# mbjd/binaural-audio-synthesis

Measured on AMD Instinct MI355X. Metric: stereo samples/sec, 256 concurrent moving sources @44.1kHz mixed to one stereo pair (x real-time in x_realtime), higher is better.
Workload: dtype f32

## Files before the change

binaural-audio-synthesis_amd/csrc/bas_fused.h:

```cpp
#pragma once
#include "bas_internal.h"
#include "bas_plan.h"
#include "bas_window.h"
#include "bas_tail.h"

#ifndef FZ_ASM
#define FZ_ASM 1
#endif
#if FZ_ASM
#ifndef BAS_FIR_ASM_INC
#define BAS_FIR_ASM_INC "bas_fir_asm.inc"
#endif
#include BAS_FIR_ASM_INC
#ifndef BAS_FIR_ONCE_ASM_INC
#define BAS_FIR_ONCE_ASM_INC "bas_fir_once_asm.inc"
#endif
#include BAS_FIR_ONCE_ASM_INC
#else
template <int XR>
__device__ __forceinline__ void ffa_row_step_asm(f32x32 &, f32x32 &, f32x2 &, f32x32 &, unsigned, unsigned, float, unsigned) {}
#endif

struct FzArgs {
    long x_stride;
    int n_src;
    long T_in;
    int K, S, L, Lp;
    int n_chunks;
    int s_pow2;
    float invK, invS;
    long units_total;
    int units_per_wg, parts_per_wg;
    int nslots;
    int spw;
    unsigned packed_bytes;
    int direct;
    int accumulate;
    long T_out;
    unsigned *ctl;
    int tail_mode;
#ifdef BAS_DIAG
    int inject;
#endif
};

__device__ __forceinline__ bool fz_wait_handover(volatile unsigned *flag, unsigned pass_id, const FzArgs &A) {
    int limit = 1 << 22;
#ifdef BAS_DIAG
    if (A.inject) limit = 1 << 8;
#endif
    int spins = 0;
    while ((unsigned)__builtin_amdgcn_readfirstlane(*flag) != pass_id) {
        if (++spins >= limit) {
            if ((threadIdx.x & 63) == 0 && A.ctl) bas_report_status(A.ctl, BAS_STATUS_HANDOVER_TIMEOUT, blockIdx.x);
            return false;
        }
        __builtin_amdgcn_s_sleep(1);
    }
    return true;
}

__device__ __forceinline__ bool fz_inject(const FzArgs &A) {
#ifdef BAS_DIAG
    return A.inject != 0;
#else
    return false;
#endif
}

__device__ __forceinline__ BasTail fz_tail(const FzArgs &A, float *y, unsigned int *peak_bits) {
    BasTail T;
    T.ctl = A.ctl;
    T.wgpeak = reinterpret_cast<float *>(A.ctl + BAS_CTL_WORDS);
    T.y = y;
    T.n = 2 * A.T_out;
    T.peak = reinterpret_cast<float *>(peak_bits);
    T.n_wg = gridDim.x;
    T.normalize = 0;
    return T;
}

__device__ __forceinline__ void fz_pair_ears(const f32x4 &h, f32x2 &ta, f32x2 &tb) {
    const auto s0 = __builtin_amdgcn_permlane32_swap(__float_as_uint(h.z), __float_as_uint(h.x), false, false);
    const auto s1 = __builtin_amdgcn_permlane32_swap(__float_as_uint(h.w), __float_as_uint(h.y), false, false);
    ta = f32x2{__uint_as_float(s0[0]), __uint_as_float(s0[1])};
    tb = f32x2{__uint_as_float(s1[0]), __uint_as_float(s1[1])};
}


#ifndef FS_UNIT_BLOCK
#define FS_UNIT_BLOCK 1
#endif
#define BAS_FS_MAXEV 6
size_t bas_fs_lds_bytes(int nslots);
int bas_fs_unit_len(int Lp);
hipError_t bas_fs_launch(const FzArgs &A, const float *x, float *slab, const float *packed, const unsigned *plans, float *y,
                         unsigned int *peak_bits, int n_wg, size_t lds_bytes, hipStream_t st, hipEvent_t eb, hipEvent_t ee);

#define BAS_FQ_MAXEV 3
size_t bas_fq_lds_bytes(int nslots);
hipError_t bas_fq_launch(const FzArgs &A, const float *x, float *slab, const float *packed, const unsigned *plans, float *y,
                         unsigned int *peak_bits, int n_wg, size_t lds_bytes, hipStream_t st, hipEvent_t eb, hipEvent_t ee);
```

binaural-audio-synthesis_amd/csrc/bas_fused_split.hip:

```cpp
#include "bas_fused.h"
#include <stdlib.h>

#ifndef FS_PSPLIT
#define FS_PSPLIT 1
#endif
#ifndef FS_TAPS_ONCE
#define FS_TAPS_ONCE 1
#endif
#ifndef FS_STAGER_PRIO
#define FS_STAGER_PRIO 3
#endif
#ifndef FS_FILTER_PRIO
#define FS_FILTER_PRIO 0
#endif

#ifdef BAS_STAMPS
__device__ unsigned long long bas_fs_stamps[1024 * 8 * 8];
#define FS_NOW() __builtin_amdgcn_s_memrealtime()
#else
#define FS_NOW() 0ull
#endif

#if FZ_ASM
template <int UNITLEN, int NSUB = 1, int PSPLIT = 0>
__global__ __launch_bounds__(512, 1) void bas_render_fs_kernel(
    FzArgs A, const float *__restrict__ x,
    float *__restrict__ slab,
    const float *__restrict__ packed,
    const unsigned *__restrict__ plans,
    float *__restrict__ y, unsigned int *__restrict__ peak_bits) {
    constexpr int NW = 4;
    constexpr int THREADS = 64 * NW;
    constexpr int TILE = 2048 * NW;
    constexpr int ROWS = TILE / 32 + HD_HALO;
    constexpr int XR = ROWS + 1;
    constexpr int NX = (ROWS * 8 + THREADS - 1) / THREADS;
    constexpr int XFLOATS = 8 * XR * 4;
    constexpr int MAXEV = BAS_FS_MAXEV;
    constexpr int PL4 = WIN_PL4;
    constexpr int NPV = (MAXEV * PL4 + 63) / 64;
    static_assert(XR == 261, "bas_fir_asm.inc holds the row step for this x-image stride");
    extern __shared__ f32x4 lds4[];
    const int buf4 = (XFLOATS + ((A.nslots * HD_SLOT + 3) & ~3)) / 4;
    f32x4 *pl_base = lds4 + 2 * buf4;
    f32x4 *bnd = pl_base + NW * (MAXEV * PL4);
    volatile unsigned *flags = reinterpret_cast<volatile unsigned *>(bnd + NW * 64);

    const int tid0 = threadIdx.x;
    const int lane0 = tid0 & 63;
    const int wv8 = __builtin_amdgcn_readfirstlane(tid0 >> 6);
    const bool stager = wv8 >= NW;
    const int wv = wv8 & (NW - 1);

    const WinWalk W = win_walk(A.units_total, A.units_per_wg, A.Lp);
    const long n_pass = W.n_pass;
    if (!A.direct && peak_bits && blockIdx.x == 0 && tid0 == 0) *peak_bits = 0u;
    if (n_pass <= 0) {
        if (A.direct && A.tail_mode) bas_tail<2 * THREADS>(fz_tail(A, y, peak_bits), 0.f);
        return;
    }
    unsigned wmax_bits = 0u;
    if (tid0 < NW) flags[tid0] = 0u;
    __syncthreads();

    const long first_tile = W.unit0 / A.n_src;
    long tile = first_tile;
    int s = (int)(W.unit0 - first_tile * A.n_src);
    int sg = 0;
    WinGeo G = win_geo<TILE>(tile, sg, A.K, A.Lp);
    auto advance = [&]() {
        const WinPos N = win_next(tile, s, sg, W.nseg, A.n_src);
        if (N.tile != tile || N.sg != sg) G = win_geo<TILE>(N.tile, N.sg, A.K, A.Lp);
        tile = N.tile, s = N.s, sg = N.sg;
    };
#ifdef BAS_STAMPS
    unsigned long long st_work = 0, st_wait = 0, st_clk = 0;
    const unsigned long long st_begin = FS_NOW(), st_begin_clk = __builtin_amdgcn_s_memtime();
#endif

    if (!stager) {
        if (FS_FILTER_PRIO) __builtin_amdgcn_s_setprio(FS_FILTER_PRIO);
        static_assert(!PSPLIT || (NSUB == 1 && UNITLEN != 0), "the P split exists for the unit blocks of subchunks >= 32");
        f32x32 accA, accB, accP;
        f32x2 accB16 = f32x2{0.f, 0.f};
        f32x16 accPA, accPB, accPP;
        f32x2 accPB8 = f32x2{0.f, 0.f};
#pragma unroll
        for (int i = 0; i < 32; ++i) accA[i] = accB[i] = accP[i] = 0.f;
#pragma unroll
        for (int i = 0; i < 16; ++i) accPA[i] = accPB[i] = accPP[i] = 0.f;
        float *slab_wg = slab + (long)blockIdx.x * A.parts_per_wg * 2 * TILE;
        auto flush = [&](long t) {
            f32x2 acc[32];
            if constexpr (PSPLIT) {
#pragma unroll
                for (int r = 0; r < 8; ++r) {
                    const f32x2 a = f32x2{accPA[2 * r], accPA[2 * r + 1]}, b0 = f32x2{accPB[2 * r], accPB[2 * r + 1]};
                    const f32x2 b1 = r < 7 ? f32x2{accPB[2 * r + 2], accPB[2 * r + 3]} : accPB8;
                    const f32x2 pp = f32x2{accPP[2 * r], accPP[2 * r + 1]};
                    const f32x2 pe = a + b0, po = (pp - a) - b1;
                    accP[4 * r] = pe.x; accP[4 * r + 1] = pe.y;
                    accP[4 * r + 2] = po.x; accP[4 * r + 3] = po.y;
                }
            }
            win_combine_pinned(acc, accA, accB, accB16, accP);
            win_zero_pinned(accA, accB, accB16, accP);
            if constexpr (PSPLIT) {
#pragma unroll
                for (int i = 0; i < 16; ++i) accPA[i] = accPB[i] = accPP[i] = 0.f;
                accPB8 = f32x2{0.f, 0.f};
            }
            if (A.direct) {
                const long n0 = t * TILE + 2048 * wv + 32 * lane0;
                const float lmax = win_store_row_direct(acc, y, A.T_out, n0, A.accumulate);
                if (A.tail_mode) {
                    const unsigned b = win_wave_max_bits(lmax);
                    wmax_bits = b > wmax_bits ? b : wmax_bits;
                } else if (peak_bits) {
                    bas_wave_peak_max(lmax, peak_bits);
                }
                return;
            }
            win_store_row_slab(acc, slab_wg + (t - first_tile) * 2 * TILE + 2048 * wv + 32 * lane0, TILE);
        };
        long open_tile = -1;
        long addr_tile = -1;
        int addr_buf = 0;
        unsigned tapv[5] = {0u, 0u, 0u, 0u, 0u}, xrow4 = 0u;
        float alv[5] = {0.f, 0.f, 0.f, 0.f, 0.f}, blv[5] = {0.f, 0.f, 0.f, 0.f, 0.f};
        float wnv[4] = {0.f, 0.f, 0.f, 0.f};
        const unsigned buf_bytes = 16u * (unsigned)buf4;
        for (long pid = 0; pid < n_pass; ++pid) {
            int tid = tid0;
            asm volatile("" : "+v"(tid));
            const int lane = tid & 63;
#ifdef BAS_STAMPS
            const unsigned long long t0 = FS_NOW();
#endif
            if (tile != open_tile) {
                if (open_tile >= 0) flush(open_tile);
                open_tile = tile;
            }
            if constexpr (UNITLEN != 0) {
                const int cur_buf = (int)(pid & 1);
                const long akey = tile * W.nseg + sg;
                if (akey == addr_tile && cur_buf != addr_buf) {
                    const unsigned delta = cur_buf ? buf_bytes : 0u - buf_bytes;
#pragma unroll
                    for (int r = 0; r < 5; ++r) tapv[r] += delta;
                    xrow4 += delta;
                    addr_buf = cur_buf;
                }
                if (akey != addr_tile) {
                    addr_tile = akey;
                    addr_buf = cur_buf;
                    const unsigned bufb = (unsigned)reinterpret_cast<uintptr_t>(lds4 + cur_buf * buf4);
                    const int row_out = 64 * wv + lane + G.halo;
                    int sl, m_in;
                    win_row_slot(G.mo0 + 32 * row_out, A.K, A.invK, sl, m_in);
                    xrow4 = bufb + 16u * (unsigned)(row_out - 4);
                    unsigned tap = bufb + 4u * (unsigned)(XFLOATS + sl * HD_SLOT - 32 * 4);
#pragma unroll
                    for (int r = 0; r < 5; ++r) {
                        alv[r] = win_weight(m_in, A.S, A.s_pow2, A.invK, A.invS);
                        if constexpr (NSUB == 2) blv[r] = win_weight(m_in + 16, A.S, A.s_pow2, A.invK, A.invS);
                        tapv[r] = tap;
                        m_in -= 32;
                        const bool wrap = m_in < 0;
                        if constexpr (PSPLIT == 2) { if (r < 4) wnv[r] = wrap ? 1.f : alv[r]; }
                        m_in += wrap ? A.K : 0;
                        tap += 32u * 16u - (wrap ? 4u * (unsigned)HD_SLOT : 0u);
                    }
                }
            }
#ifdef BAS_STAMPS
            const unsigned long long t1 = FS_NOW();
#endif
            __syncthreads();
#ifdef BAS_STAMPS
            const unsigned long long t2 = FS_NOW();
#endif
            const f32x4 *xs4 = lds4 + (pid & 1) * buf4;
            const float *hd = reinterpret_cast<const float *>(xs4) + XFLOATS;
            const int Lseg = G.Lseg, halo = G.halo;
#ifdef BAS_STAMPS
            const unsigned long long c0 = __builtin_amdgcn_s_memtime();
#endif
            if constexpr (UNITLEN != 0) {
                if constexpr (PSPLIT == 2) {
                    const unsigned tapo[4] = {tapv[1], tapv[2], tapv[3], tapv[4]};
                    const float wov[4] = {alv[1], alv[2], alv[3], alv[4]};
                    ffa_unitp1_asm<XR, UNITLEN>(accA, accB, accPA, accPB, accPB8, accPP, accB16, xrow4, tapo, wnv, wov);
                } else if constexpr (PSPLIT)
                    ffa_unitp_asm<XR, UNITLEN>(accA, accB, accPA, accPB, accPB8, accPP, accB16, xrow4, tapv, alv);
                else if constexpr (NSUB == 4)
                    ffa_unit4_asm<XR, UNITLEN>(accA, accB, accB16, accP, xrow4, tapv, alv, (float)A.S * A.invK);
                else if constexpr (NSUB == 2)
                    ffa_unit2_asm<XR, UNITLEN>(accA, accB, accB16, accP, xrow4, tapv, alv, blv);
                else
                    ffa_unit_asm<XR, UNITLEN>(accA, accB, accB16, accP, xrow4, tapv, alv);
                (void)hd; (void)Lseg; (void)halo;
            } else {
                const int row_out = 64 * wv + lane + halo;
                int sl, m_in;
                win_row_slot(G.mo0 + 32 * row_out, A.K, A.invK, sl, m_in);
                const f32x4 *xrow = xs4 + row_out;
#pragma unroll 1
                for (int rp = 0; rp <= halo; ++rp) {
                    const float al = win_weight(m_in, A.S, A.s_pow2, A.invK, A.invS);
                    const unsigned mk = win_octet_mask(rp, Lseg);
                    ffa_row_step_asm<XR>(accA, accB, accB16, accP, (unsigned)reinterpret_cast<uintptr_t>(xrow),
                                         (unsigned)reinterpret_cast<uintptr_t>(hd + sl * HD_SLOT + (32 * rp - 32) * 4), al, mk);
                    xrow -= 1;
                    win_row_up(A.K, sl, m_in);
                }
            }
#ifdef BAS_STAMPS
            st_clk += __builtin_amdgcn_s_memtime() - c0;
            st_work += (t1 - t0) + (FS_NOW() - t2);
            st_wait += t2 - t1;
#endif
            advance();
        }
        flush(open_tile);
    } else {
        __builtin_amdgcn_s_setprio(FS_STAGER_PRIO);
        const __amdgpu_buffer_rsrc_t tab =
            __builtin_amdgcn_make_buffer_rsrc(const_cast<float *>(packed), 0, (int)A.packed_bytes, 0x00020000);
        const unsigned L4 = 4u * (unsigned)A.L;
        const int n_ir = A.nslots + 1, base = n_ir / NW, rem = n_ir - base * NW;
        const int slot_a = rfl(wv * base + (wv < rem ? wv : rem));
        const int slot_b = rfl(slot_a + base + (wv < rem ? 1 : 0));
        const int n_ev = slot_a < slot_b ? slot_b - slot_a : 0;
        const bool need_next = n_ev > 0 && slot_b <= A.nslots;
        f32x4 *plw = pl_base + wv * (MAXEV * PL4);
        const int tid = tid0 - THREADS;
        const int lane = tid & 63;
        const int half = lane >> 5;
        const int tq = 4 * (lane & 31) + (lane < 32 ? 2 : 0);
        const unsigned v16 = 16u * (unsigned)tid, l16 = 16u * (unsigned)lane;
        const bool all_live = A.L == A.Lp;
        for (long pid = 0; pid < n_pass; ++pid) {
#ifdef BAS_STAMPS
            const unsigned long long t0 = FS_NOW();
#endif
#ifndef FS_NO_STAGE
            f32x4 *xs4 = lds4 + (pid & 1) * buf4;
            float *hd = reinterpret_cast<float *>(xs4) + XFLOATS;
            const int seg0 = G.seg0, Lseg = G.Lseg, nrows = G.nrows;
            const long xbase = G.xbase;
            f32x4 pv[NPV], xv[NX];
            {
                const f32x4 *pl_src = reinterpret_cast<const f32x4 *>(plans) + (long)s * (A.n_chunks + 1) * PL4;
                const int c_first = rfl(G.c0 + slot_a);
                if (c_first >= 0 && c_first + n_ev - 1 <= A.n_chunks) {
                    const __amdgpu_buffer_rsrc_t pr = __builtin_amdgcn_make_buffer_rsrc(
                        const_cast<f32x4 *>(pl_src + (long)c_first * PL4), 0, n_ev * PL4 * 16, 0x00020000);
#pragma unroll
                    for (int r = 0; r < NPV; ++r)
                        pv[r] = __builtin_bit_cast(f32x4, __builtin_amdgcn_raw_buffer_load_b128(pr, (int)l16, 1024 * r, 2));
                } else {
#pragma unroll
                    for (int r = 0; r < NPV; ++r) {
                        pv[r] = __builtin_nontemporal_load(win_plan_piece(pl_src, lane, r, n_ev, c_first, A.n_chunks));
                    }
                }
            }
            const WinXBounds XB = win_x_bounds(xbase, A.T_in);
            const bool x_inside = win_x_inside<NX, THREADS>(XB);
            {
                const float *xwin = x + (long)s * A.x_stride + xbase;
                if (x_inside) {
                    const __amdgpu_buffer_rsrc_t xr = __builtin_amdgcn_make_buffer_rsrc(const_cast<float *>(xwin), 0,
                                                                                        16 * NX * THREADS, 0x00020000);
#pragma unroll
                    for (int j = 0; j < NX; ++j)
                        xv[j] = __builtin_bit_cast(f32x4, __builtin_amdgcn_raw_buffer_load_b128(xr, (int)v16, 16 * THREADS * j, 2));
                } else {
                    asm volatile("" ::: "memory");
#pragma unroll
                    for (int j = 0; j < NX; ++j) {
                        int i = 4 * (tid + j * THREADS);
                        i = i < XB.lo ? XB.lo : i;
                        i = i > XB.hi - 4 ? XB.hi - 4 : i;
                        xv[j] = __builtin_nontemporal_load(reinterpret_cast<const f32x4 *>(xwin + i));
                    }
                }
            }
            const unsigned pass_id = (unsigned)pid + 1u;
#pragma unroll
            for (int r = 0; r < NPV; ++r)
                if (lane + 64 * r < n_ev * PL4) plw[lane + 64 * r] = pv[r];
            {
                f32x4 *xcol = xs4 + (tid & 7) * XR + (tid >> 3);
                if (!x_inside) {
                    asm volatile("" ::: "memory");
#pragma unroll
                    for (int j = 0; j < NX; ++j) {
                        const int e = 4 * (tid + j * THREADS);
                        if (!(e >= XB.lo && e < XB.hi)) xv[j] = f32x4{0.f, 0.f, 0.f, 0.f};
                    }
                }
#pragma unroll
                for (int j = 0; j < NX; ++j) {
                    if ((j + 1) * THREADS <= (TILE / 32 + 1) * 8 || tid + j * THREADS < nrows * 8) xcol[32 * j] = xv[j];
                }
            }
            __builtin_amdgcn_wave_barrier();

            {
                const int m = seg0 + 4 * (lane & 31);
                const int m_c = m < A.L ? m : A.L - 1;
                const unsigned m4 = 4u * (unsigned)m_c;
                const f32x4 live = f32x4{m < A.L ? 1.f : 0.f, m + 1 < A.L ? 1.f : 0.f, m + 2 < A.L ? 1.f : 0.f,
                                         m + 3 < A.L ? 1.f : 0.f};
                const f32x4 *pl = plw + half * (BAS_PLANS_WORDS / 4);
                f32x4 *dst = reinterpret_cast<f32x4 *>(hd) + slot_a * (HD_SLOT / 4) + tq;
                FzHalf ha, hb;
                f32x2 pa = f32x2{0.f, 0.f}, pb = pa;
                const f32x4 *pl_last = pl + (n_ev > 0 ? n_ev - 1 : 0) * PL4;
                if (n_ev > 0) fz_issue<0>(tab, pl, m4, L4, ha);
                for (int i = 0; i < n_ev; ++i) {
                    const f32x4 *pl_next = pl + PL4 < pl_last ? pl + PL4 : pl_last;
                    fz_issue<1>(tab, pl, m4, L4, hb);
                    f32x4 h = fz_finish<0>(pl, ha, f32x4{0.f, 0.f, 0.f, 0.f});
                    fz_issue<0>(tab, pl_next, m4, L4, ha);
                    h = fz_finish<1>(pl, hb, h);
                    if (!all_live) h *= live;
                    if (i == 0 && wv > 0) {
                        bnd[wv * 64 + lane] = h;
                        __builtin_amdgcn_fence(__ATOMIC_RELEASE, "workgroup");
                        if (lane == 0 && !fz_inject(A)) flags[wv] = pass_id;
                    }
                    f32x2 ca, cb;
                    fz_pair_ears(h, ca, cb);
                    if (i > 0) {
                        const f32x2 da = ca - pa, db = cb - pb;
                        if (tq < Lseg) {
                            dst[0] = f32x4{pa.x, pa.y, da.x, da.y};
                            dst[1] = f32x4{pb.x, pb.y, db.x, db.y};
                        }
                        dst += HD_SLOT / 4;
                    }
                    pa = ca;
                    pb = cb;
                    pl = pl_next;
                }
                if (need_next) {
                    const bool got = fz_wait_handover(flags + wv + 1, pass_id, A);
                    __builtin_amdgcn_fence(__ATOMIC_ACQUIRE, "workgroup");
                    f32x4 nx = bnd[(wv + 1) * 64 + lane];
                    if (!got) nx = f32x4{__builtin_nanf(""), __builtin_nanf(""), __builtin_nanf(""), __builtin_nanf("")};
                    f32x2 ca, cb;
                    fz_pair_ears(nx, ca, cb);
                    const f32x2 da = ca - pa, db = cb - pb;
                    if (tq < Lseg) {
                        dst[0] = f32x4{pa.x, pa.y, da.x, da.y};
                        dst[1] = f32x4{pb.x, pb.y, db.x, db.y};
                    }
                }
            }
#endif
#ifdef BAS_STAMPS
            asm volatile("s_waitcnt vmcnt(0) lgkmcnt(0)" ::: "memory");
            const unsigned long long t1 = FS_NOW();
#endif
            __syncthreads();
#ifdef BAS_STAMPS
            st_work += t1 - t0;
            st_wait += FS_NOW() - t1;
#endif
            advance();
        }
    }
    if (A.direct && A.tail_mode) bas_tail<2 * THREADS>(fz_tail(A, y, peak_bits), __uint_as_float(wmax_bits));
#ifdef BAS_STAMPS
    if (lane0 == 0 && blockIdx.x < 1024) {
        unsigned long long *d = bas_fs_stamps + (blockIdx.x * 8 + wv8) * 8;
        d[0] = st_work;
        d[1] = st_wait;
        d[2] = st_clk;
        d[3] = __builtin_amdgcn_s_memtime() - st_begin_clk;
        d[6] = FS_NOW() - st_begin;
        d[7] = (unsigned long long)n_pass;
    }
#endif
}

#ifdef BAS_STAMPS
extern "C" int bas_debug_read_fs_stamps(unsigned long long *host, size_t count) {
    return (int)hipMemcpyFromSymbol(host, HIP_SYMBOL(bas_fs_stamps), count * sizeof(unsigned long long));
}
#endif

#endif

int bas_fs_unit_len(int Lp) {
    return FS_UNIT_BLOCK && (Lp == 104 || (Lp > 0 && Lp % 128 == 0)) ? (Lp == 104 ? 104 : 128) : 0;
}

size_t bas_fs_lds_bytes(int nslots) {
    const int rows = 8192 / 32 + HD_HALO;
    return (size_t)(2 * (8 * (rows + 1) * 4 + ((nslots * HD_SLOT + 3) & ~3)) + 4 * BAS_FS_MAXEV * 2 * BAS_PLANS_WORDS + 4 * 64 * 4 + 4) *
           sizeof(float);
}

hipError_t bas_fs_launch(const FzArgs &A, const float *x, float *slab, const float *packed, const unsigned *plans, float *y,
                         unsigned int *peak_bits, int n_wg, size_t lds_bytes, hipStream_t st, hipEvent_t eb, hipEvent_t ee) {
#if FZ_ASM
    typedef void (*fs_fn)(FzArgs, const float *, float *, const float *, const unsigned *, float *, unsigned int *);
    const int ul = bas_fs_unit_len(A.Lp);
#if FS_PSPLIT && FS_TAPS_ONCE
    fs_fn fn = ul == 128 ? bas_render_fs_kernel<128, 1, 2> : ul == 104 ? bas_render_fs_kernel<104, 1, 2> : bas_render_fs_kernel<0>;
#ifdef BAS_DIAG
    {
        const char *once = getenv("BAS_FS_TAPS_ONCE");
        if (once && atoi(once) == 0 && ul != 0) fn = ul == 128 ? bas_render_fs_kernel<128, 1, 1> : bas_render_fs_kernel<104, 1, 1>;
    }
#endif
#elif FS_PSPLIT
    fs_fn fn = ul == 128 ? bas_render_fs_kernel<128, 1, 1> : ul == 104 ? bas_render_fs_kernel<104, 1, 1> : bas_render_fs_kernel<0>;
#else
    fs_fn fn = ul == 128 ? bas_render_fs_kernel<128> : ul == 104 ? bas_render_fs_kernel<104> : bas_render_fs_kernel<0>;
#endif
    if (A.S == 16 || A.S == 8) {
        if (ul == 0) return hipErrorNotSupported;
        fn = A.S == 16 ? (ul == 128 ? bas_render_fs_kernel<128, 2> : bas_render_fs_kernel<104, 2>)
                       : (ul == 128 ? bas_render_fs_kernel<128, 4> : bas_render_fs_kernel<104, 4>);
    }
    hipError_t e = bas_allow_full_lds(reinterpret_cast<const void *>(fn));
    if (e != hipSuccess) return e;
    if (eb) (void)hipEventRecord(eb, st);
    hipLaunchKernelGGL(fn, dim3(n_wg), dim3(512), lds_bytes, st, A, x, slab, packed, plans, y, peak_bits);
    if (ee) (void)hipEventRecord(ee, st);
    return hipSuccess;
#else
    return hipErrorNotSupported;
#endif
}
```

Baseline: 741.5 million.

## Replace per-pass workgroup barrier with LDS handover flags and rotate stager slot deal

Filter waves and stager waves no longer meet at a full workgroup barrier each pass. Instead they signal through per-wave LDS 'staged' and 'drained' counters, so stagers can run ahead into the double buffer while filters are still consuming the previous pass. The stager deal of IR slots now rotates between passes, so the wave that must wait on a neighbour's boundary changes from pass to pass. This trades barrier stalls for spin-wait polling and more delicate memory-ordering logic, and the old barrier path stays available under a diagnostic switch.

```diff
diff --git a/binaural-audio-synthesis_amd/csrc/bas_fused.h b/binaural-audio-synthesis_amd/csrc/bas_fused.h
--- a/binaural-audio-synthesis_amd/csrc/bas_fused.h
+++ b/binaural-audio-synthesis_amd/csrc/bas_fused.h
@@ -41,23 +41,45 @@
     int tail_mode;
 #ifdef BAS_DIAG
     int inject;
+    int fs_barrier;
 #endif
 };
 
+#define FZ_HANDOVER_SPINS (1 << 22)
+
+__device__ __forceinline__ void fz_report_handover_timeout(const FzArgs &A);
 __device__ __forceinline__ bool fz_wait_handover(volatile unsigned *flag, unsigned pass_id, const FzArgs &A) {
-    int limit = 1 << 22;
+    int limit = FZ_HANDOVER_SPINS;
 #ifdef BAS_DIAG
     if (A.inject) limit = 1 << 8;
 #endif
     int spins = 0;
     while ((unsigned)__builtin_amdgcn_readfirstlane(*flag) != pass_id) {
         if (++spins >= limit) {
-            if ((threadIdx.x & 63) == 0 && A.ctl) bas_report_status(A.ctl, BAS_STATUS_HANDOVER_TIMEOUT, blockIdx.x);
+            fz_report_handover_timeout(A);
             return false;
         }
         __builtin_amdgcn_s_sleep(1);
     }
     return true;
+}
+
+__device__ __forceinline__ bool fz_wait_handover4(volatile unsigned *words, unsigned pass_id) {
+    const unsigned base = (unsigned)reinterpret_cast<uintptr_t>(words);
+    int spins = 0;
+    for (;;) {
+        unsigned v = base + 4u * (threadIdx.x & 3u);
+        asm volatile("ds_read_b32 %0, %0\n\ts_waitcnt lgkmcnt(0)" : "+v"(v) : : "memory");
+        if (__builtin_amdgcn_ballot_w64(v < pass_id) == 0ull) return true;
+        if (++spins >= FZ_HANDOVER_SPINS) return false;
+        __builtin_amdgcn_s_sleep(1);
+    }
+}
+__device__ __forceinline__ void fz_store_handover(volatile unsigned *word, unsigned pass_id) {
+    asm volatile("s_waitcnt lgkmcnt(0)\n\tds_write_b32 %0, %1" ::"v"((unsigned)reinterpret_cast<uintptr_t>(word)), "v"(pass_id) : "memory");
+}
+__device__ __forceinline__ void fz_report_handover_timeout(const FzArgs &A) {
+    if ((threadIdx.x & 63) == 0 && A.ctl) bas_report_status(A.ctl, BAS_STATUS_HANDOVER_TIMEOUT, blockIdx.x);
 }
 
 __device__ __forceinline__ bool fz_inject(const FzArgs &A) {
diff --git a/binaural-audio-synthesis_amd/csrc/bas_fused_split.hip b/binaural-audio-synthesis_amd/csrc/bas_fused_split.hip
--- a/binaural-audio-synthesis_amd/csrc/bas_fused_split.hip
+++ b/binaural-audio-synthesis_amd/csrc/bas_fused_split.hip
@@ -1,5 +1,6 @@
 #include "bas_fused.h"
 #include <stdlib.h>
+#include <string.h>
 
 #ifndef FS_PSPLIT
 #define FS_PSPLIT 1
@@ -13,6 +14,32 @@
 #ifndef FS_FILTER_PRIO
 #define FS_FILTER_PRIO 0
 #endif
+
+#ifndef FS_HANDOVER_FLAGS
+#define FS_HANDOVER_FLAGS 1
+#endif
+#ifndef FS_ROTATE_DEAL
+#define FS_ROTATE_DEAL 1
+#endif
+
+__device__ __forceinline__ bool fs_by_barrier(const FzArgs &A) {
+#if !FS_HANDOVER_FLAGS
+    return true;
+#elif defined(BAS_DIAG)
+    return A.fs_barrier != 0;
+#else
+    return false;
+#endif
+}
+
+__host__ __device__ __forceinline__ int fs_deal_rank(int wv, long pass) {
+    return FS_ROTATE_DEAL ? (wv + 2 * (int)(pass & 1)) & 3 : wv;
+}
+__host__ __device__ __forceinline__ void fs_deal(int nslots, int rank, int &slot_a, int &slot_b) {
+    const int n_ir = nslots + 1, base = n_ir / 4, rem = n_ir - base * 4;
+    slot_a = rank * base + (rank < rem ? rank : rem);
+    slot_b = slot_a + base + (rank < rem ? 1 : 0);
+}
 
 #ifdef BAS_STAMPS
 __device__ unsigned long long bas_fs_stamps[1024 * 8 * 8];
@@ -45,6 +72,9 @@
     f32x4 *pl_base = lds4 + 2 * buf4;
     f32x4 *bnd = pl_base + NW * (MAXEV * PL4);
     volatile unsigned *flags = reinterpret_cast<volatile unsigned *>(bnd + NW * 64);
+    volatile unsigned *staged = flags + NW, *drained = flags + 2 * NW;
+    static_assert(NW == 4, "fz_wait_handover4 waits for four words");
+    const bool by_barrier = fs_by_barrier(A);
 
     const int tid0 = threadIdx.x;
     const int lane0 = tid0 & 63;
@@ -60,7 +90,7 @@
         return;
     }
     unsigned wmax_bits = 0u;
-    if (tid0 < NW) flags[tid0] = 0u;
+    if (tid0 < 3 * NW) flags[tid0] = 0u;
     __syncthreads();
 
     const long first_tile = W.unit0 / A.n_src;
@@ -124,6 +154,7 @@
             win_store_row_slab(acc, slab_wg + (t - first_tile) * 2 * TILE + 2048 * wv + 32 * lane0, TILE);
         };
         long open_tile = -1;
+        bool ho_ok = true;
         long addr_tile = -1;
         int addr_buf = 0;
         unsigned tapv[5] = {0u, 0u, 0u, 0u, 0u}, xrow4 = 0u;
@@ -176,7 +207,12 @@
 #ifdef BAS_STAMPS
             const unsigned long long t1 = FS_NOW();
 #endif
-            __syncthreads();
+            if (by_barrier) {
+                __syncthreads();
+            } else {
+                ho_ok &= fz_wait_handover4(staged, (unsigned)pid + 1u);
+                __builtin_amdgcn_fence(__ATOMIC_ACQUIRE, "workgroup");
+            }
 #ifdef BAS_STAMPS
             const unsigned long long t2 = FS_NOW();
 #endif
@@ -215,6 +251,10 @@
                     win_row_up(A.K, sl, m_in);
                 }
             }
+            if (!by_barrier) {
+                __builtin_amdgcn_fence(__ATOMIC_RELEASE, "workgroup");
+                if ((tid0 & 63) == 0) fz_store_handover(drained + wv, (unsigned)pid + 1u);
+            }
 #ifdef BAS_STAMPS
             st_clk += __builtin_amdgcn_s_memtime() - c0;
             st_work += (t1 - t0) + (FS_NOW() - t2);
@@ -223,16 +263,12 @@
             advance();
         }
         flush(open_tile);
+        if (!ho_ok) fz_report_handover_timeout(A);
     } else {
         __builtin_amdgcn_s_setprio(FS_STAGER_PRIO);
         const __amdgpu_buffer_rsrc_t tab =
             __builtin_amdgcn_make_buffer_rsrc(const_cast<float *>(packed), 0, (int)A.packed_bytes, 0x00020000);
         const unsigned L4 = 4u * (unsigned)A.L;
-        const int n_ir = A.nslots + 1, base = n_ir / NW, rem = n_ir - base * NW;
-        const int slot_a = rfl(wv * base + (wv < rem ? wv : rem));
-        const int slot_b = rfl(slot_a + base + (wv < rem ? 1 : 0));
-        const int n_ev = slot_a < slot_b ? slot_b - slot_a : 0;
-        const bool need_next = n_ev > 0 && slot_b <= A.nslots;
         f32x4 *plw = pl_base + wv * (MAXEV * PL4);
         const int tid = tid0 - THREADS;
         const int lane = tid & 63;
@@ -242,8 +278,24 @@
         const bool all_live = A.L == A.Lp;
         for (long pid = 0; pid < n_pass; ++pid) {
 #ifdef BAS_STAMPS
+            const unsigned long long tw = FS_NOW();
+#endif
+            const unsigned pass_id = (unsigned)pid + 1u;
+            if (!by_barrier && pid > 0) {
+                bool ok = fz_wait_handover4(staged, pass_id - 1u);
+                if (pid > 1) ok &= fz_wait_handover4(drained, pass_id - 2u);
+                if (!ok) fz_report_handover_timeout(A);
+                __builtin_amdgcn_fence(__ATOMIC_ACQUIRE, "workgroup");
+            }
+#ifdef BAS_STAMPS
             const unsigned long long t0 = FS_NOW();
 #endif
+            const int rank = fs_deal_rank(wv, pid);
+            int deal_a, deal_b;
+            fs_deal(A.nslots, rank, deal_a, deal_b);
+            const int slot_a = rfl(deal_a), slot_b = rfl(deal_b);
+            const int n_ev = slot_a < slot_b ? slot_b - slot_a : 0;
+            const bool need_next = n_ev > 0 && slot_b <= A.nslots;
 #ifndef FS_NO_STAGE
             f32x4 *xs4 = lds4 + (pid & 1) * buf4;
             float *hd = reinterpret_cast<float *>(xs4) + XFLOATS;
@@ -287,7 +339,6 @@
                     }
                 }
             }
-            const unsigned pass_id = (unsigned)pid + 1u;
 #pragma unroll
             for (int r = 0; r < NPV; ++r)
                 if (lane + 64 * r < n_ev * PL4) plw[lane + 64 * r] = pv[r];
@@ -327,10 +378,10 @@
                     fz_issue<0>(tab, pl_next, m4, L4, ha);
                     h = fz_finish<1>(pl, hb, h);
                     if (!all_live) h *= live;
-                    if (i == 0 && wv > 0) {
-                        bnd[wv * 64 + lane] = h;
+                    if (i == 0 && rank > 0) {
+                        bnd[rank * 64 + lane] = h;
                         __builtin_amdgcn_fence(__ATOMIC_RELEASE, "workgroup");
-                        if (lane == 0 && !fz_inject(A)) flags[wv] = pass_id;
+                        if (lane == 0 && !fz_inject(A)) flags[rank] = pass_id;
                     }
                     f32x2 ca, cb;
                     fz_pair_ears(h, ca, cb);
@@ -347,9 +398,9 @@
                     pl = pl_next;
                 }
                 if (need_next) {
-                    const bool got = fz_wait_handover(flags + wv + 1, pass_id, A);
+                    const bool got = fz_wait_handover(flags + rank + 1, pass_id, A);
                     __builtin_amdgcn_fence(__ATOMIC_ACQUIRE, "workgroup");
-                    f32x4 nx = bnd[(wv + 1) * 64 + lane];
+                    f32x4 nx = bnd[(rank + 1) * 64 + lane];
                     if (!got) nx = f32x4{__builtin_nanf(""), __builtin_nanf(""), __builtin_nanf(""), __builtin_nanf("")};
                     f32x2 ca, cb;
                     fz_pair_ears(nx, ca, cb);
@@ -365,10 +416,15 @@
             asm volatile("s_waitcnt vmcnt(0) lgkmcnt(0)" ::: "memory");
             const unsigned long long t1 = FS_NOW();
 #endif
-            __syncthreads();
+            if (by_barrier) {
+                __syncthreads();
+            } else {
+                __builtin_amdgcn_fence(__ATOMIC_RELEASE, "workgroup");
+                if (lane == 0) fz_store_handover(staged + wv, pass_id);
+            }
 #ifdef BAS_STAMPS
             st_work += t1 - t0;
-            st_wait += FS_NOW() - t1;
+            st_wait += (t0 - tw) + (FS_NOW() - t1);
 #endif
             advance();
         }
@@ -401,14 +457,29 @@
 
 size_t bas_fs_lds_bytes(int nslots) {
     const int rows = 8192 / 32 + HD_HALO;
-    return (size_t)(2 * (8 * (rows + 1) * 4 + ((nslots * HD_SLOT + 3) & ~3)) + 4 * BAS_FS_MAXEV * 2 * BAS_PLANS_WORDS + 4 * 64 * 4 + 4) *
+    return (size_t)(2 * (8 * (rows + 1) * 4 + ((nslots * HD_SLOT + 3) & ~3)) + 4 * BAS_FS_MAXEV * 2 * BAS_PLANS_WORDS + 4 * 64 * 4 + 3 * 4) *
            sizeof(float);
 }
 
-hipError_t bas_fs_launch(const FzArgs &A, const float *x, float *slab, const float *packed, const unsigned *plans, float *y,
+#ifdef BAS_DIAG
+extern "C" int bas_debug_fs_deal(int nslots, int wave, long pass, int *slot_a, int *slot_b) {
+    const int rank = fs_deal_rank(wave, pass);
+    fs_deal(nslots, rank, *slot_a, *slot_b);
+    return rank;
+}
+#endif
+
+hipError_t bas_fs_launch(const FzArgs &A0, const float *x, float *slab, const float *packed, const unsigned *plans, float *y,
                          unsigned int *peak_bits, int n_wg, size_t lds_bytes, hipStream_t st, hipEvent_t eb, hipEvent_t ee) {
 #if FZ_ASM
     typedef void (*fs_fn)(FzArgs, const float *, float *, const float *, const unsigned *, float *, unsigned int *);
+    FzArgs A = A0;
+#ifdef BAS_DIAG
+    {
+        const char *ho = getenv("BAS_FS_HANDOVER");
+        A.fs_barrier = ho && strcmp(ho, "barrier") == 0;
+    }
+#endif
     const int ul = bas_fs_unit_len(A.Lp);
 #if FS_PSPLIT && FS_TAPS_ONCE
     fs_fn fn = ul == 128 ? bas_render_fs_kernel<128, 1, 2> : ul == 104 ? bas_render_fs_kernel<104, 1, 2> : bas_render_fs_kernel<0>;
```

Result: slower. 723.8 million (-2.4%).
